# bdaiinstitute/vlfm

Measured on AMD Instinct MI355X. Metric: env-steps/s (VLM+value-map update), 640x480 RGB-D, higher is better.
Workload: dtype f16 ViT-g (f32 accumulate) + f32 Q-Former (split-f16, 22-bit); f32 confidence + f64 value maps; 1 GPU; configs[1] step x resident envs: BLIP-2 ITC + ValueMap+ObstacleMap+sort_waypoints; envs_per_gpu=256, global_envs=256, map=1000x1000 @ 20 px/m, parallelism=env-sharded x1, tuned_gemms=True, vit_gemm=hip:fc1, attention=hip

## Files before the change

vlfm_amd/csrc/gemm_f16.hip:

```cpp
#include <hip/hip_runtime.h>
#include <stdint.h>

#include "../../include/vlfm_amd.h"
#include "gelu_f16.h"
#include "profile.h"
#include "status.h"

namespace vlfm {

typedef _Float16 half8 __attribute__((ext_vector_type(8)));
typedef _Float16 half4 __attribute__((ext_vector_type(4)));
typedef float floatx4 __attribute__((ext_vector_type(4)));
typedef float f32x16 __attribute__((ext_vector_type(16)));

constexpr int GB = 256;
constexpr int GK = 64;
constexpr int ROWB = GK * 2;
constexpr int OPER = GB * ROWB;
constexpr int BUF = 2 * OPER;
constexpr int EPI_ROW = 272;
constexpr int EPI_WAVE = 64 * EPI_ROW;
constexpr int GEMM_LDS = 8 * EPI_WAVE > 2 * BUF ? 8 * EPI_WAVE : 2 * BUF;
enum { EPI_BIAS = 0, EPI_BIAS_GELU = 1, EPI_ACCUM = 2,
       EPI_PAIR_F32 = 3 };

struct GemmArgs {
    const _Float16* x;
    const _Float16* w;
    const _Float16* bias;
    _Float16* c;
    int M, N, K;
    int tiles_m, tiles_n;
    int group_m;
    int split_ragged;
};

using lds_ptr = __attribute__((address_space(3))) unsigned char*;
using gbl_ptr = const __attribute__((address_space(1))) unsigned char*;

template <int EPI, int BAL, int SYNC = 2>
struct Gemm8p {
    static constexpr int SLOT = 128 * ROWB;
    static constexpr int KBUF = 4 * SLOT;

    const GemmArgs& a;
    lds_ptr lds;
    const unsigned char* smem;
    int wave, lane;
    bool half;
    bool active;
    uint32_t voff[4][2];
    uint32_t rdP[2], rdQ[2];
    half8 fp[4][2], fq0[BAL ? 2 : 1][2][2], fq1[2][2];
    floatx4 acc[8][4];

    __device__ Gemm8p(const GemmArgs& a_, unsigned char* smem_, int m0, int n0) : a(a_), lds((lds_ptr)smem_), smem(smem_) {
        const int tid = threadIdx.x;
        lane = tid & 63;
        wave = __builtin_amdgcn_readfirstlane(tid >> 6);
        const int wn = wave >> 2, wm = wave & 3;
        half = false;
        active = n0 + wn * (half ? 64 : 128) < a.N;
        offsets(m0, n0, voff);
        const int r16 = lane & 15, swz = (r16 >> 1) & 7, s0 = lane >> 4;
        const uint32_t bp = (uint32_t)(wn * 64 + r16) * ROWB + (uint32_t)((s0 ^ swz) << 4);
        const uint32_t bq = (uint32_t)(wm * 32 + r16) * ROWB + (uint32_t)((s0 ^ swz) << 4);
        rdP[0] = bp; rdP[1] = bp ^ 64u;
        rdQ[0] = bq; rdQ[1] = bq ^ 64u;
        zero_acc();
    }
    __device__ inline void zero_acc() {
#pragma unroll
        for (int i = 0; i < 8; i++)
#pragma unroll
            for (int j = 0; j < 4; j++) acc[i][j] = floatx4{0.f, 0.f, 0.f, 0.f};
    }
    __device__ inline void kill_fragments() {
        const half8 z = {(_Float16)0.f, (_Float16)0.f, (_Float16)0.f, (_Float16)0.f, (_Float16)0.f, (_Float16)0.f, (_Float16)0.f, (_Float16)0.f};
#pragma unroll
        for (int f = 0; f < 4; f++) { fp[f][0] = z; fp[f][1] = z; }
#pragma unroll
        for (int g = 0; g < 2; g++)
#pragma unroll
            for (int k = 0; k < 2; k++) {
                fq1[g][k] = z;
#pragma unroll
                for (int q = 0; q < (BAL ? 2 : 1); q++) fq0[q][g][k] = z;
            }
    }
    __device__ inline void offsets(int m0, int n0, uint32_t (&vo)[4][2]) const {
        const int sub = lane >> 3, p = lane & 7;
#pragma unroll
        for (int j = 0; j < 2; j++) {
            const int rho = (wave * 2 + j) * 8 + sub;
            const int s = p ^ ((rho >> 1) & 7);
#pragma unroll
            for (int h = 0; h < 2; h++) {
                const int rq = min(m0 + (rho >> 5) * 64 + h * 32 + (rho & 31), a.M - 1);
                const int rp = min(n0 + (half ? rho + h * 128 : (rho >> 6) * 128 + h * 64 + (rho & 63)), a.N - 1);
                vo[2 * h][j] = (uint32_t)rq * (uint32_t)a.K * 2u + (uint32_t)s * 16u;
                vo[2 * h + 1][j] = (uint32_t)rp * (uint32_t)a.K * 2u + (uint32_t)s * 16u;
            }
        }
    }

    template <int SLOT_ID>
    __device__ inline void stage_at(int b, int t, const uint32_t (&vo)[4][2]) {
        const unsigned char* base = reinterpret_cast<const unsigned char*>((SLOT_ID & 1) ? a.w : a.x) + (size_t)t * (GK * 2);
#pragma unroll
        for (int j = 0; j < 2; j++) {
            const int dst = __builtin_amdgcn_readfirstlane(b * KBUF + SLOT_ID * SLOT + (wave * 2 + j) * 1024);
            __builtin_amdgcn_global_load_lds((gbl_ptr)(base + vo[SLOT_ID][j]), lds + dst, 16, 0, 0);
        }
    }
    template <int SLOT_ID>
    __device__ inline void stage(int b, int t) { stage_at<SLOT_ID>(b, t, voff); }
    template <int B, int SLOT_ID>
    __device__ inline void read_p() {
#pragma unroll
        for (int kk = 0; kk < 2; kk++)
#pragma unroll
            for (int f = 0; f < 4; f++)
                fp[f][kk] = *reinterpret_cast<const half8*>(smem + B * KBUF + SLOT_ID * SLOT + f * 16 * ROWB + rdP[kk]);
    }
    template <int B, int SLOT_ID>
    __device__ inline void read_q(half8 (&fq)[2][2]) {
#pragma unroll
        for (int kk = 0; kk < 2; kk++)
#pragma unroll
            for (int g = 0; g < 2; g++)
                fq[g][kk] = *reinterpret_cast<const half8*>(smem + B * KBUF + SLOT_ID * SLOT + g * 16 * ROWB + rdQ[kk]);
    }
    template <int PI, int QJ>
    __device__ inline void mma(const half8 (&fq)[2][2]) {
#pragma unroll
        for (int kk = 0; kk < 2; kk++)
#pragma unroll
            for (int f = 0; f < 4; f++)
#pragma unroll
                for (int g = 0; g < 2; g++)
                    acc[PI * 4 + f][QJ * 2 + g] =
                        __builtin_amdgcn_mfma_f32_16x16x32_f16(fp[f][kk], fq[g][kk], acc[PI * 4 + f][QJ * 2 + g], 0, 0, 0);
    }
    static __device__ inline void bar() {
        __builtin_amdgcn_s_barrier();
        asm volatile("" ::: "memory");
    }
    template <int PI, int QJ>
    __device__ inline void compute(const half8 (&fq)[2][2], bool work = true) {
        bar();
        __builtin_amdgcn_s_waitcnt(0xC07F);
        __builtin_amdgcn_sched_barrier(0);
        if (active && work) {
            __builtin_amdgcn_s_setprio(1);
            mma<PI, QJ>(fq);
            __builtin_amdgcn_s_setprio(0);
        }
        __builtin_amdgcn_sched_barrier(0);
        if (SYNC == 2) bar();
    }

    template <int B>
    __device__ inline void tile(int t, int NT) {
        constexpr int QS = BAL ? B : 0;
        if (active) {
            if (!BAL) read_q<B, 0>(fq0[QS]);
            read_p<B, 1>();
        }
        __builtin_amdgcn_sched_barrier(0);
        if (t + 1 < NT) stage<2>(B ^ 1, t + 1);
        compute<0, 0>(fq0[QS]);
        if (active) read_q<B, 2>(fq1);
        __builtin_amdgcn_sched_barrier(0);
        if (t + 1 < NT) stage<3>(B ^ 1, t + 1);
        compute<0, 1>(fq1);
        if (active) read_p<B, 3>();
        __builtin_amdgcn_sched_barrier(0);
        if (t + 2 < NT) {
            stage<0>(B, t + 2);
            if (BAL) __builtin_amdgcn_s_waitcnt(0x0F78);
        } else if (BAL) {
            __builtin_amdgcn_s_waitcnt(0x0F76);
        }
        compute<1, 1>(fq1);
        if (BAL && active && t + 1 < NT) read_q<B ^ 1, 0>(fq0[BAL ? (B ^ 1) : 0]);
        __builtin_amdgcn_sched_barrier(0);
        if (t + 2 < NT) {
            stage<1>(B, t + 2);
            __builtin_amdgcn_s_waitcnt(0x0F74);
        } else {
            __builtin_amdgcn_s_waitcnt(0x0F70);
        }
        compute<1, 0>(fq0[QS]);
    }
};

__host__ __device__ inline void tile_of(const GemmArgs& a, int bid, int& tm, int& tn) {
    const int nwg = a.tiles_m * a.tiles_n;
    const int xcd = bid & 7, idx = bid >> 3;
    const int tail_cols = a.N - (a.tiles_n - 1) * GB;
    const bool ragged = a.tiles_n > 1 && tail_cols <= GB / 2;
    const int ncols = ragged ? a.tiles_n - 1 : a.tiles_n;
    const int nfull = a.tiles_m * ncols, nhalf = nwg - nfull;
    const int qf = nfull >> 3, rf = nfull & 7, qh = nhalf >> 3, rh = nhalf & 7;
    const int myfull = qf + (xcd < rf ? 1 : 0);
    if (idx < myfull) {
        const int f = xcd * qf + min(xcd, rf) + idx;
        const int GM = a.group_m;
        const int per_group = GM * ncols, grp = f / per_group, in = f - grp * per_group;
        const int rows = min(GM, a.tiles_m - grp * GM);
        tn = in / rows;
        tm = grp * GM + (in - tn * rows);
    } else {
        int before = 0;
        for (int x = 0; x < xcd; x++) before += (((x - rf) & 7) < rh) ? 1 : 0;
        tm = xcd * qh + before + (idx - myfull);
        tn = a.tiles_n - 1;
    }
}

constexpr int EPI2_ROW = 144;
constexpr int EPI2_WAVE = 64 * EPI2_ROW;
constexpr int PBIAS_OFF = GEMM_LDS;
constexpr int GEMM_LDS_P = GEMM_LDS + 512;

__device__ __forceinline__ half8 add_half8(half8 a, const half8 b) {
#pragma unroll
    for (int e = 0; e < 8; e++) a[e] = (_Float16)((float)a[e] + (float)b[e]);
    return a;
}
template <int EPI, int H>
__device__ __forceinline__ void epi2_pass(const floatx4 (&acc)[8][4], const half4 (&bias4)[8], unsigned char* stg, int g4, int c16, int rsub,
                                 int chunk, half8 (&v)[8]) {
#pragma unroll
    for (int ii = 0; ii < 4; ii++) {
        constexpr int I0 = H * 4;
        const float b0 = (float)bias4[I0 + ii][0], b1 = (float)bias4[I0 + ii][1], b2 = (float)bias4[I0 + ii][2], b3 = (float)bias4[I0 + ii][3];
#pragma unroll
        for (int j = 0; j < 4; j++) {
            float v0 = acc[I0 + ii][j][0] + b0, v1 = acc[I0 + ii][j][1] + b1, v2 = acc[I0 + ii][j][2] + b2, v3 = acc[I0 + ii][j][3] + b3;
            if (EPI == EPI_BIAS_GELU) gelu_erf4(v0, v1, v2, v3);
            const half4 hv = {(_Float16)v0, (_Float16)v1, (_Float16)v2, (_Float16)v3};
            *reinterpret_cast<half4*>(stg + (j * 16 + c16) * EPI2_ROW + (ii * 16 + g4) * 2) = hv;
        }
    }
    __builtin_amdgcn_s_waitcnt(0xC07F);
#pragma unroll
    for (int it = 0; it < 8; it++) v[it] = *reinterpret_cast<const half8*>(stg + (it * 8 + rsub) * EPI2_ROW + chunk * 16);
}
template <int P>
__device__ __forceinline__ void epi_pair_pass(const floatx4 (&acc)[8][4], const floatx4 (&bias4)[4], unsigned char* stg, int g4, int c16,
                                              int rsub, int chunk, floatx4 (&v)[8]) {
#pragma clang fp contract(off)
#pragma unroll
    for (int i2 = 0; i2 < 2; i2++) {
        constexpr int I0 = 2 * P;
#pragma unroll
        for (int j = 0; j < 4; j++) {
            floatx4 r;
#pragma unroll
            for (int e = 0; e < 4; e++) {
                const float low = acc[4 + I0 + i2][j][e] * 0x1p-11f;
                const float mid = bias4[I0 + i2][e] + low;
                r[e] = acc[I0 + i2][j][e] + mid;
            }
            *reinterpret_cast<floatx4*>(stg + (j * 16 + c16) * EPI2_ROW + (i2 * 16 + g4) * 4) = r;
        }
    }
    __builtin_amdgcn_s_waitcnt(0xC07F);
#pragma unroll
    for (int it = 0; it < 8; it++) v[it] = *reinterpret_cast<const floatx4*>(stg + (it * 8 + rsub) * EPI2_ROW + chunk * 16);
}
__device__ __forceinline__ void stage_bias(const GemmArgs& a, lds_ptr lds, int wave, int lane, int n_first) {
    if (a.bias != nullptr && wave == 0 && lane < 32) {
        const _Float16* src = a.bias + min(n_first + lane * 8, a.N - 8);
        __builtin_amdgcn_global_load_lds((gbl_ptr)src, lds + PBIAS_OFF, 16, 0, 0);
    }
}

struct WorkList {
    int nwg, first_split, nitems;
    __host__ __device__ WorkList(int nwg_, int grid, bool allow = true) : nwg(nwg_) {
        const int left = nwg > grid ? nwg % grid : 0;
        const bool split = allow && left > 0 && 2 * left <= grid;
        first_split = split ? nwg - left : nwg;
        nitems = nwg + (split ? left : 0);
    }
    __host__ __device__ void item(int w, int& pos, int& half) const {
        if (w < first_split) { pos = w; half = -1; }
        else { const int j = w - first_split; pos = first_split + (j >> 1); half = j & 1; }
    }
};

template <int EPI>
__global__ __launch_bounds__(512) void gemm_f16_8pp_kernel(GemmArgs a) {
    extern __shared__ __attribute__((aligned(16))) unsigned char smem[];
    using G = Gemm8p<EPI, 1, 2>;
    const int stride = gridDim.x;
    const WorkList work(a.tiles_m * a.tiles_n, stride, a.split_ragged != 0);
    int bid = blockIdx.x;
    int tm, tn, pos, half;
    work.item(bid, pos, half);
    tile_of(a, pos, tm, tn);
    int m0 = tm * GB, n0 = tn * GB;
    G g(a, smem, m0, n0);
    g.active = g.active && (half < 0 || half == (g.wave >> 2));
    const int NT = a.K / GK;
    const int wave = g.wave, lane = g.lane, wn = wave >> 2, wm = wave & 3, late = wn;
    const int g4 = (lane >> 4) * 4, c16 = lane & 15;
    const int rsub = lane >> 3, chunk = lane & 7;
    unsigned char* stg = smem + G::KBUF + wave * EPI2_WAVE;
    const bool has_bias = a.bias != nullptr;
    stage_bias(a, g.lds, wave, lane, n0);
    g.template stage<0>(0, 0); g.template stage<1>(0, 0); g.template stage<2>(0, 0); g.template stage<3>(0, 0);
    if (NT > 1) {
        g.template stage<0>(1, 1); g.template stage<1>(1, 1);
        __builtin_amdgcn_s_waitcnt(0x0F74);
    } else {
        __builtin_amdgcn_s_waitcnt(0x0F70);
    }
    g.bar();
    for (;;) {
        g.kill_fragments();
        if (late) g.bar();
        if (g.active) g.template read_q<0, 0>(g.fq0[0]);
        for (int t = 0; t < NT; t += 2) {
            g.template tile<0>(t, NT);
            if (t + 1 < NT) g.template tile<1>(t + 1, NT);
        }
        if (!late) g.bar();

        half4 bias4[EPI == EPI_PAIR_F32 ? 1 : 8];
        floatx4 biasf[EPI == EPI_PAIR_F32 ? 4 : 1];
        if constexpr (EPI == EPI_PAIR_F32) {
#pragma unroll
            for (int i = 0; i < 4; i++) {
                const floatx4 ld = *reinterpret_cast<const floatx4*>(smem + PBIAS_OFF + (wn * 64 + i * 16 + g4) * 4);
                biasf[i] = has_bias ? ld : floatx4{0.f, 0.f, 0.f, 0.f};
            }
        } else {
#pragma unroll
            for (int i = 0; i < 8; i++) {
                const half4 ld = *reinterpret_cast<const half4*>(smem + PBIAS_OFF + (wn * 128 + i * 16 + g4) * 2);
                bias4[i] = has_bias ? ld : half4{(_Float16)0.f, (_Float16)0.f, (_Float16)0.f, (_Float16)0.f};
            }
        }
        __builtin_amdgcn_sched_barrier(0);
        const int nbid = bid + stride;
        const bool more = nbid < work.nitems;
        const bool store = g.active;
        work.item(more ? nbid : bid, pos, half);
        tile_of(a, pos, tm, tn);
        const int m1 = tm * GB, n1 = tn * GB;
        uint32_t von[4][2];
        g.offsets(m1, n1, von);
        g.template stage_at<0>(0, 0, von); g.template stage_at<1>(0, 0, von);
        g.template stage_at<2>(0, 0, von); g.template stage_at<3>(0, 0, von);
        __builtin_amdgcn_sched_barrier(0);
        half8 old[EPI == EPI_ACCUM ? 16 : 1];
        if (EPI == EPI_ACCUM) {
#pragma unroll
            for (int h = 0; h < 2; h++)
#pragma unroll
                for (int it = 0; it < 8; it++) {
                    const int m = min(m0 + wm * 64 + it * 8 + rsub, a.M - 1);
                    const int n = max(min(n0 + wn * 128 + h * 64 + chunk * 8, a.N - 8), 0);
                    old[h * 8 + it] = *reinterpret_cast<const half8*>(a.c + (size_t)m * a.N + n);
                }
        }
        __builtin_amdgcn_sched_barrier(0);
        if constexpr (EPI == EPI_PAIR_F32) {
            (void)bias4; (void)old;
            floatx4 p0[8], p1[8];
            epi_pair_pass<0>(g.acc, biasf, stg, g4, c16, rsub, chunk, p0);
            epi_pair_pass<1>(g.acc, biasf, stg, g4, c16, rsub, chunk, p1);
            __builtin_amdgcn_sched_barrier(0);
            __builtin_amdgcn_s_waitcnt(0x0F70);
            __builtin_amdgcn_sched_barrier(0);
            const int nblk = n0 + wn * 128;
            if (store && nblk + 128 <= a.N) {
                float* ob = reinterpret_cast<float*>(a.c) + (size_t)(nblk >> 7) * (size_t)a.M * 64 + chunk * 4;
#pragma unroll
                for (int it = 0; it < 8; it++) {
                    const int m = m0 + wm * 64 + it * 8 + rsub;
                    if (m < a.M) *reinterpret_cast<floatx4*>(ob + (size_t)m * 64) = p0[it];
                }
#pragma unroll
                for (int it = 0; it < 8; it++) {
                    const int m = m0 + wm * 64 + it * 8 + rsub;
                    if (m < a.M) *reinterpret_cast<floatx4*>(ob + (size_t)m * 64 + 32) = p1[it];
                }
            }
        } else {
        (void)biasf;
        half8 v0[8], v1[8];
        epi2_pass<EPI, 0>(g.acc, bias4, stg, g4, c16, rsub, chunk, v0);
        epi2_pass<EPI, 1>(g.acc, bias4, stg, g4, c16, rsub, chunk, v1);
        if (EPI == EPI_ACCUM) {
#pragma unroll
            for (int it = 0; it < 8; it++) {
                v0[it] = add_half8(v0[it], old[it]);
                v1[it] = add_half8(v1[it], old[8 + it]);
            }
        }
        __builtin_amdgcn_sched_barrier(0);
        __builtin_amdgcn_s_waitcnt(0x0F70);
        __builtin_amdgcn_sched_barrier(0);
        {
            const int n = n0 + wn * 128 + chunk * 8;
            if (store && n + 8 <= a.N) {
#pragma unroll
                for (int it = 0; it < 8; it++) {
                    const int m = m0 + wm * 64 + it * 8 + rsub;
                    if (m < a.M) *reinterpret_cast<half8*>(a.c + (size_t)m * a.N + n) = v0[it];
                }
            }
            if (store && n + 64 + 8 <= a.N) {
#pragma unroll
                for (int it = 0; it < 8; it++) {
                    const int m = m0 + wm * 64 + it * 8 + rsub;
                    if (m < a.M) *reinterpret_cast<half8*>(a.c + (size_t)m * a.N + n + 64) = v1[it];
                }
            }
        }
        }
        if (!more) break;
        bid = nbid; m0 = m1; n0 = n1;
#pragma unroll
        for (int s = 0; s < 4; s++) { g.voff[s][0] = von[s][0]; g.voff[s][1] = von[s][1]; }
        g.active = n0 + wn * 128 < a.N && (half < 0 || half == wn);
        g.zero_acc();
        g.bar();
        stage_bias(a, g.lds, wave, lane, n0);
        if (NT > 1) { g.template stage<0>(1, 1); g.template stage<1>(1, 1); }
    }
}


}

using namespace vlfm;

template <int EPI>
static int launch_gemm(const GemmArgs& a, hipStream_t stream) {
    const void* fn = reinterpret_cast<const void*>(gemm_f16_8pp_kernel<EPI>);
    static LdsOptIn optp;
    if (!optp.ensure(fn, GEMM_LDS_P)) return fail(VLFM_ERR_HIP, "gemm_f16_nt: cannot opt in to the LDS size");
    const int n_cu = device_cu_count() & ~7;
    const int nwg = a.tiles_m * a.tiles_n;
    const dim3 grid(nwg < n_cu ? nwg : n_cu), block(512);
    VLFM_TIMED(EPI == EPI_BIAS ? "gemm_f16_8pp_kernel<0>" : EPI == EPI_BIAS_GELU ? "gemm_f16_8pp_kernel<1>" :
               EPI == EPI_ACCUM ? "gemm_f16_8pp_kernel<2>" : "gemm_f16_8pp_kernel<3>", stream);
    VLFM_KLAUNCH((gemm_f16_8pp_kernel<EPI>), grid, block, GEMM_LDS_P, stream, a);
    return check_launch("gemm_f16_8pp_kernel");
}

extern "C" int vlfm_gemm_f16_nt(const void* d_x, const void* d_w, const void* d_bias, void* d_c, int m, int n, int k,
                                int epilogue, void* stream) {
    if (m == 0 || n == 0) return VLFM_OK;
    if (!d_x || !d_w || !d_c || m < 0 || n < 0 || k <= 0 || (k % GK) != 0 || (n % 8) != 0 || epilogue < 0 || epilogue > 2)
        return fail(VLFM_ERR_INVALID, "gemm_f16_nt: K must be a multiple of 64, N of 8, epilogue 0, 1 or 2");
    if ((size_t)m * (size_t)k * 2 >= (1ull << 32) || (size_t)n * (size_t)k * 2 >= (1ull << 32))
        return fail(VLFM_ERR_INVALID, "gemm_f16_nt: an operand of 4 GB or more (32-bit byte offsets inside an operand)");
    GemmArgs a;
    a.x = (const _Float16*)d_x; a.w = (const _Float16*)d_w; a.bias = (const _Float16*)d_bias; a.c = (_Float16*)d_c;
    a.M = m; a.N = n; a.K = k;
    a.tiles_m = (m + GB - 1) / GB; a.tiles_n = (n + GB - 1) / GB;
    a.group_m = 4;
    a.split_ragged = 1;
    if (epilogue == 0) return launch_gemm<EPI_BIAS>(a, (hipStream_t)stream);
    if (epilogue == 1) return launch_gemm<EPI_BIAS_GELU>(a, (hipStream_t)stream);
    return launch_gemm<EPI_ACCUM>(a, (hipStream_t)stream);
}

extern "C" int vlfm_gemm_f16_pair_f32_nt(const void* d_x, const void* d_w_pair, const void* d_bias_f32, void* d_out, int m, int n_out,
                                         int k, void* stream) {
    if (m == 0 || n_out == 0) return VLFM_OK;
    if (!d_x || !d_w_pair || !d_out || m < 0 || n_out < 0 || k <= 0 || (k % GK) != 0 || (n_out % 64) != 0)
        return fail(VLFM_ERR_INVALID, "gemm_f16_pair_f32_nt: K and N_out must be multiples of 64");
    if ((size_t)m * (size_t)k * 2 >= (1ull << 32) || (size_t)n_out * (size_t)k * 4 >= (1ull << 32))
        return fail(VLFM_ERR_INVALID, "gemm_f16_pair_f32_nt: an operand of 4 GB or more (32-bit byte offsets inside an operand)");
    GemmArgs a;
    a.x = (const _Float16*)d_x; a.w = (const _Float16*)d_w_pair;
    a.bias = (const _Float16*)d_bias_f32;
    a.c = (_Float16*)d_out;
    a.M = m; a.N = 2 * n_out; a.K = k;
    a.tiles_m = (m + GB - 1) / GB; a.tiles_n = (a.N + GB - 1) / GB;
    a.group_m = 4;
    a.split_ragged = 1;
    return launch_gemm<EPI_PAIR_F32>(a, (hipStream_t)stream);
}

extern "C" int vlfm_gemm_f16_tile_order(int m, int n, int group_m, int* out, int capacity_pairs) {
    if (m <= 0 || n <= 0 || !out) return fail(VLFM_ERR_INVALID, "gemm_f16_tile_order: m, n > 0 and an output array");
    GemmArgs a{};
    a.M = m; a.N = n; a.K = GK;
    a.tiles_m = (m + GB - 1) / GB; a.tiles_n = (n + GB - 1) / GB;
    a.group_m = group_m > 0 ? group_m : 4;
    const int nwg = a.tiles_m * a.tiles_n;
    if (capacity_pairs < nwg) return fail(VLFM_ERR_INVALID, "gemm_f16_tile_order: output array too small");
    for (int b = 0; b < nwg; b++) tile_of(a, b, out[2 * b], out[2 * b + 1]);
    return nwg;
}

extern "C" int vlfm_gemm_f16_work_items(int m, int n, int grid, int* out, int capacity_pairs) {
    if (m <= 0 || n <= 0 || grid <= 0 || !out) return fail(VLFM_ERR_INVALID, "gemm_f16_work_items: m, n, grid > 0 and an output array");
    const int nwg = ((m + GB - 1) / GB) * ((n + GB - 1) / GB);
    const WorkList work(nwg, grid < nwg ? grid : nwg);
    if (capacity_pairs < work.nitems) return fail(VLFM_ERR_INVALID, "gemm_f16_work_items: output array too small");
    for (int w = 0; w < work.nitems; w++) work.item(w, out[2 * w], out[2 * w + 1]);
    return work.nitems;
}
```

Measured before the change: 1757 env-steps/s.

## Balance full and half tiles per XCD with a cost model and precomputed per-WG work lists

Reworks how GEMM tiles are distributed across XCDs and workgroups. A host-side cost model (full tile cost 10, half tile cost 6) decides how many ragged half-width tiles each XCD and each workgroup gets, so that per-workgroup work is evened out. Each workgroup also precomputes its persistent-loop item list into LDS at kernel start, replacing the per-iteration work.item/tile_of arithmetic. This adds LDS usage, a prologue pass and a tile-count cap, and the new indexing logic is intricate, with a risk of scheduling mistakes.

Result: no change. 1744 env-steps/s (-0.8%).

```diff
diff --git a/vlfm_amd/csrc/gemm_f16.hip b/vlfm_amd/csrc/gemm_f16.hip
--- a/vlfm_amd/csrc/gemm_f16.hip
+++ b/vlfm_amd/csrc/gemm_f16.hip
@@ -33,6 +33,7 @@
     int tiles_m, tiles_n;
     int group_m;
     int split_ragged;
+    int xk_long, xk_short, xe_long, xe_short;
 };
 
 using lds_ptr = __attribute__((address_space(3))) unsigned char*;
@@ -195,26 +196,69 @@
     }
 };
 
+constexpr int COST_FULL = 10, COST_HALF = 6;
+
+__host__ __device__ inline void fill_halves(int n_long, int c_long, int n_short, int halves, int (&k)[2], int (&e)[2]) {
+    int k0 = 0, k1 = 0, e0 = 0, e1 = 0;
+    const int c_short = c_long - 1, step = COST_FULL - COST_HALF;
+    while (halves > 0) {
+        const int v0 = n_long > 0 && k0 < c_long ? COST_FULL * c_long - step * k0 : -1;
+        const int v1 = n_short > 0 && k1 < c_short ? COST_FULL * c_short - step * k1 : -1;
+        if (v0 < 0 && v1 < 0) break;
+        if (v0 >= v1) {
+            if (halves >= n_long) { k0++; halves -= n_long; } else { e0 = halves; halves = 0; }
+        } else {
+            if (halves >= n_short) { k1++; halves -= n_short; } else { e1 = halves; halves = 0; }
+        }
+    }
+    k[0] = k0; k[1] = k1; e[0] = e0; e[1] = e1;
+}
+
+struct TileCounts {
+    int nwg, ncols, nfull, nhalf;
+    __host__ __device__ explicit TileCounts(const GemmArgs& a) {
+        nwg = a.tiles_m * a.tiles_n;
+        const int tail_cols = a.N - (a.tiles_n - 1) * GB;
+        const bool ragged = a.tiles_n > 1 && tail_cols <= GB / 2;
+        ncols = ragged ? a.tiles_n - 1 : a.tiles_n;
+        nfull = a.tiles_m * ncols;
+        nhalf = nwg - nfull;
+    }
+};
+__host__ inline void set_xcd_shares(GemmArgs& a) {
+    const TileCounts t(a);
+    int k[2], e[2];
+    fill_halves(t.nwg & 7, (t.nwg >> 3) + 1, 8 - (t.nwg & 7), t.nhalf, k, e);
+    a.xk_long = k[0]; a.xk_short = k[1]; a.xe_long = e[0]; a.xe_short = e[1];
+}
+struct XcdShare {
+    int n, nfull, full0, half0;
+    __host__ __device__ XcdShare(const GemmArgs& a, int x) {
+        const int nwg = a.tiles_m * a.tiles_n, nl = nwg & 7, q = nwg >> 3;
+        const bool lng = x < nl;
+        const int r = lng ? x : x - nl;
+        n = q + (lng ? 1 : 0);
+        const int nh = lng ? a.xk_long + (r < a.xe_long ? 1 : 0) : a.xk_short + (r < a.xe_short ? 1 : 0);
+        half0 = lng ? x * a.xk_long + min(x, a.xe_long)
+                    : nl * a.xk_long + a.xe_long + r * a.xk_short + min(r, a.xe_short);
+        nfull = n - nh;
+        full0 = x * q + min(x, nl) - half0;
+    }
+};
+
 __host__ __device__ inline void tile_of(const GemmArgs& a, int bid, int& tm, int& tn) {
-    const int nwg = a.tiles_m * a.tiles_n;
     const int xcd = bid & 7, idx = bid >> 3;
-    const int tail_cols = a.N - (a.tiles_n - 1) * GB;
-    const bool ragged = a.tiles_n > 1 && tail_cols <= GB / 2;
-    const int ncols = ragged ? a.tiles_n - 1 : a.tiles_n;
-    const int nfull = a.tiles_m * ncols, nhalf = nwg - nfull;
-    const int qf = nfull >> 3, rf = nfull & 7, qh = nhalf >> 3, rh = nhalf & 7;
-    const int myfull = qf + (xcd < rf ? 1 : 0);
-    if (idx < myfull) {
-        const int f = xcd * qf + min(xcd, rf) + idx;
+    const XcdShare sh(a, xcd);
+    if (idx < sh.nfull) {
+        const TileCounts t(a);
+        const int f = sh.full0 + idx;
         const int GM = a.group_m;
-        const int per_group = GM * ncols, grp = f / per_group, in = f - grp * per_group;
+        const int per_group = GM * t.ncols, grp = f / per_group, in = f - grp * per_group;
         const int rows = min(GM, a.tiles_m - grp * GM);
         tn = in / rows;
         tm = grp * GM + (in - tn * rows);
     } else {
-        int before = 0;
-        for (int x = 0; x < xcd; x++) before += (((x - rf) & 7) < rh) ? 1 : 0;
-        tm = xcd * qh + before + (idx - myfull);
+        tm = sh.half0 + (idx - sh.nfull);
         tn = a.tiles_n - 1;
     }
 }
@@ -222,7 +266,9 @@
 constexpr int EPI2_ROW = 144;
 constexpr int EPI2_WAVE = 64 * EPI2_ROW;
 constexpr int PBIAS_OFF = GEMM_LDS;
-constexpr int GEMM_LDS_P = GEMM_LDS + 512;
+constexpr int ITEMS_OFF = GEMM_LDS + 512;
+constexpr int ITEM_CAP = 512;
+constexpr int GEMM_LDS_P = ITEMS_OFF + ITEM_CAP * 8;
 
 __device__ __forceinline__ half8 add_half8(half8 a, const half8 b) {
 #pragma unroll
@@ -279,29 +325,117 @@
 }
 
 struct WorkList {
-    int nwg, first_split, nitems;
-    __host__ __device__ WorkList(int nwg_, int grid, bool allow = true) : nwg(nwg_) {
+    int nwg, grid, first_split, nitems;
+    bool even;
+    int xcd, G, q, r, nfull, k[2], e[2];
+    __host__ __device__ WorkList(const GemmArgs& a, int grid_, int xcd_, bool allow = true) : grid(grid_), xcd(xcd_) {
+        const TileCounts t(a);
+        nwg = t.nwg;
         const int left = nwg > grid ? nwg % grid : 0;
         const bool split = allow && left > 0 && 2 * left <= grid;
         first_split = split ? nwg - left : nwg;
         nitems = nwg + (split ? left : 0);
+        G = grid >> 3; q = 0; r = 0; nfull = 0; k[0] = k[1] = e[0] = e[1] = 0;
+        even = allow && t.nhalf > 0 && (grid & 7) == 0 && nwg > grid;
+        if (!even) return;
+        q = nwg / grid;
+        for (int x = 0; x < 8; x++) {
+            const XcdShare sh(a, x);
+            if (split && sh.n - sh.nfull < (left + 7 - x) / 8) even = false;
+        }
+        if (!even) return;
+        const XcdShare sh(a, xcd);
+        nfull = sh.nfull;
+        r = sh.n - q * G;
+        fill_halves(r, q + 1, G - r, sh.n - sh.nfull, k, e);
+    }
+    __host__ __device__ int real_items(int w) const { return q + ((w >> 3) < r ? 1 : 0); }
+    __host__ __device__ int items_of(int w) const { return even ? real_items(w) : w < nitems ? (nitems - w + grid - 1) / grid : 0; }
+    __host__ __device__ bool real(int i) const {
+        if (i >= nitems) return false;
+        return !even || i / grid < real_items(i % grid);
+    }
+    __host__ __device__ int even_index(int l, int j) const {
+        const int size[4] = {e[0], r - e[0], e[1], G - r - e[1]};
+        const int halves[4] = {k[0] + 1, k[0], k[1] + 1, k[1]};
+        int fulls[4], c = 0, in = l, my_fulls = 0, my_halves = 0, fmin = q + 1;
+#pragma unroll
+        for (int i = 0, at = 0; i < 4; i++) {
+            fulls[i] = q + (i < 2 ? 1 : 0) - halves[i];
+            if (size[i] > 0 && l >= at) { c = i; in = l - at; my_fulls = fulls[i]; my_halves = halves[i]; }
+            if (size[i] > 0 && fulls[i] < fmin) fmin = fulls[i];
+            at += size[i];
+        }
+        if (j < my_fulls) {
+            int base = min(j, fmin) * G;
+            for (int jj = fmin; jj < j; jj++)
+#pragma unroll
+                for (int i = 0; i < 4; i++) base += fulls[i] > jj ? size[i] : 0;
+#pragma unroll
+            for (int i = 0; i < 4; i++) base += i < c && fulls[i] > j ? size[i] : 0;
+            return base + in;
+        }
+        int h = in * my_halves + (j - my_fulls);
+#pragma unroll
+        for (int i = 0; i < 4; i++) h += i < c ? size[i] * halves[i] : 0;
+        return nfull + h;
     }
     __host__ __device__ void item(int w, int& pos, int& half) const {
-        if (w < first_split) { pos = w; half = -1; }
-        else { const int j = w - first_split; pos = first_split + (j >> 1); half = j & 1; }
+        if (!even) {
+            const int j = w - first_split, left = nwg - first_split;
+            if (j < 0) { pos = w; half = -1; }
+            else if (((left | grid) & 7) == 0) {
+                const int row = j >> 3;
+                pos = first_split + (row >> 1) * 8 + (j & 7); half = row & 1;
+            } else { pos = first_split + (j >> 1); half = j & 1; }
+            return;
+        }
+        const int wg = w % grid, j = w / grid;
+        if (j < real_items(wg)) {
+            pos = even_index(wg >> 3, j) * 8 + xcd;
+            half = pos >= first_split ? 0 : -1;
+            return;
+        }
+        int rank = 0;
+        for (int v = 0; v < wg; v++) {
+            const int nv = (nwg >> 3) + ((v & 7) < (nwg & 7) ? 1 : 0);
+            rank += (v >> 3) < nv - q * G ? 0 : 1;
+        }
+        pos = first_split + rank;
+        half = 1;
     }
 };
+
+__device__ __noinline__ int list_items(int N, int tiles_m, int tiles_n, int group_m, int split_ragged, int xk_long, int xk_short,
+                                       int xe_long, int xe_short, uint32_t* items) {
+    GemmArgs a{};
+    a.N = N; a.tiles_m = tiles_m; a.tiles_n = tiles_n; a.group_m = group_m; a.split_ragged = split_ragged;
+    a.xk_long = xk_long; a.xk_short = xk_short; a.xe_long = xe_long; a.xe_short = xe_short;
+    const int stride = gridDim.x, w = blockIdx.x;
+    const WorkList work(a, stride, w & 7, a.split_ragged != 0);
+    const int count = work.items_of(w);
+    for (int j = threadIdx.x; j < count; j += 512) {
+        int p, h, im, in;
+        work.item(w + j * stride, p, h);
+        tile_of(a, p, im, in);
+        items[2 * j] = (uint32_t)im;
+        items[2 * j + 1] = (uint32_t)in | ((uint32_t)(h + 1) << 30);
+    }
+    return count;
+}
 
 template <int EPI>
 __global__ __launch_bounds__(512) void gemm_f16_8pp_kernel(GemmArgs a) {
     extern __shared__ __attribute__((aligned(16))) unsigned char smem[];
     using G = Gemm8p<EPI, 1, 2>;
-    const int stride = gridDim.x;
-    const WorkList work(a.tiles_m * a.tiles_n, stride, a.split_ragged != 0);
-    int bid = blockIdx.x;
-    int tm, tn, pos, half;
-    work.item(bid, pos, half);
-    tile_of(a, pos, tm, tn);
+    uint32_t* const items = reinterpret_cast<uint32_t*>(smem + ITEMS_OFF);
+    int count = list_items(a.N, a.tiles_m, a.tiles_n, a.group_m, a.split_ragged, a.xk_long, a.xk_short, a.xe_long, a.xe_short, items);
+    count = __builtin_amdgcn_readfirstlane(count);
+    __syncthreads();
+    int slot = 0;
+    int tm = __builtin_amdgcn_readfirstlane((int)items[0]), tn = __builtin_amdgcn_readfirstlane((int)items[1]);
+    int half = (tn >> 30) - 1;
+    tn &= 0x3FFFFFFF;
     int m0 = tm * GB, n0 = tn * GB;
     G g(a, smem, m0, n0);
     g.active = g.active && (half < 0 || half == (g.wave >> 2));
@@ -346,11 +480,13 @@
             }
         }
         __builtin_amdgcn_sched_barrier(0);
-        const int nbid = bid + stride;
-        const bool more = nbid < work.nitems;
+        const bool more = slot + 1 < count;
         const bool store = g.active;
-        work.item(more ? nbid : bid, pos, half);
-        tile_of(a, pos, tm, tn);
+        slot += more ? 1 : 0;
+        tm = __builtin_amdgcn_readfirstlane((int)items[2 * slot]);
+        tn = __builtin_amdgcn_readfirstlane((int)items[2 * slot + 1]);
+        half = (tn >> 30) - 1;
+        tn &= 0x3FFFFFFF;
         const int m1 = tm * GB, n1 = tn * GB;
         uint32_t von[4][2];
         g.offsets(m1, n1, von);
@@ -425,7 +561,7 @@
         }
         }
         if (!more) break;
-        bid = nbid; m0 = m1; n0 = n1;
+        m0 = m1; n0 = n1;
 #pragma unroll
         for (int s = 0; s < 4; s++) { g.voff[s][0] = von[s][0]; g.voff[s][1] = von[s][1]; }
         g.active = n0 + wn * 128 < a.N && (half < 0 || half == wn);
@@ -449,6 +585,7 @@
     const int n_cu = device_cu_count() & ~7;
     const int nwg = a.tiles_m * a.tiles_n;
     const dim3 grid(nwg < n_cu ? nwg : n_cu), block(512);
+    if (nwg / (int)grid.x + 2 > ITEM_CAP) return fail(VLFM_ERR_INVALID, "gemm_f16_nt: more than 510 tiles per workgroup");
     VLFM_TIMED(EPI == EPI_BIAS ? "gemm_f16_8pp_kernel<0>" : EPI == EPI_BIAS_GELU ? "gemm_f16_8pp_kernel<1>" :
                EPI == EPI_ACCUM ? "gemm_f16_8pp_kernel<2>" : "gemm_f16_8pp_kernel<3>", stream);
     VLFM_KLAUNCH((gemm_f16_8pp_kernel<EPI>), grid, block, GEMM_LDS_P, stream, a);
@@ -468,6 +605,7 @@
     a.tiles_m = (m + GB - 1) / GB; a.tiles_n = (n + GB - 1) / GB;
     a.group_m = 4;
     a.split_ragged = 1;
+    set_xcd_shares(a);
     if (epilogue == 0) return launch_gemm<EPI_BIAS>(a, (hipStream_t)stream);
     if (epilogue == 1) return launch_gemm<EPI_BIAS_GELU>(a, (hipStream_t)stream);
     return launch_gemm<EPI_ACCUM>(a, (hipStream_t)stream);
@@ -488,6 +626,7 @@
     a.tiles_m = (m + GB - 1) / GB; a.tiles_n = (a.N + GB - 1) / GB;
     a.group_m = 4;
     a.split_ragged = 1;
+    set_xcd_shares(a);
     return launch_gemm<EPI_PAIR_F32>(a, (hipStream_t)stream);
 }
 
@@ -497,6 +636,7 @@
     a.M = m; a.N = n; a.K = GK;
     a.tiles_m = (m + GB - 1) / GB; a.tiles_n = (n + GB - 1) / GB;
     a.group_m = group_m > 0 ? group_m : 4;
+    set_xcd_shares(a);
     const int nwg = a.tiles_m * a.tiles_n;
     if (capacity_pairs < nwg) return fail(VLFM_ERR_INVALID, "gemm_f16_tile_order: output array too small");
     for (int b = 0; b < nwg; b++) tile_of(a, b, out[2 * b], out[2 * b + 1]);
@@ -505,9 +645,20 @@
 
 extern "C" int vlfm_gemm_f16_work_items(int m, int n, int grid, int* out, int capacity_pairs) {
     if (m <= 0 || n <= 0 || grid <= 0 || !out) return fail(VLFM_ERR_INVALID, "gemm_f16_work_items: m, n, grid > 0 and an output array");
-    const int nwg = ((m + GB - 1) / GB) * ((n + GB - 1) / GB);
-    const WorkList work(nwg, grid < nwg ? grid : nwg);
-    if (capacity_pairs < work.nitems) return fail(VLFM_ERR_INVALID, "gemm_f16_work_items: output array too small");
-    for (int w = 0; w < work.nitems; w++) work.item(w, out[2 * w], out[2 * w + 1]);
-    return work.nitems;
-}
+    GemmArgs a{};
+    a.M = m; a.N = n; a.K = GK;
+    a.tiles_m = (m + GB - 1) / GB; a.tiles_n = (n + GB - 1) / GB;
+    a.group_m = 4;
+    set_xcd_shares(a);
+    const int nwg = a.tiles_m * a.tiles_n, g = grid < nwg ? grid : nwg;
+    int nitems = 0;
+    for (int x = 0; x < 8; x++) {
+        const WorkList work(a, g, x);
+        nitems = work.nitems;
+        if (capacity_pairs < nitems) return fail(VLFM_ERR_INVALID, "gemm_f16_work_items: output array too small");
+        for (int w = 0; w < nitems; w++)
+            if (!work.even || ((w % g) & 7) == x) work.item(w, out[2 * w], out[2 * w + 1]);
+        if (!work.even) break;
+    }
+    return nitems;
+}
```
